# SCoulY/MuSCLe

Measured on AMD Instinct MI355X. Metric: images/sec (whole node), MCL EfficientNet-B7 448x448 bs=32/GPU, higher is better.
Workload: dtype f32; 1 GPU; train_mcl.py loop body, step-A (epoch-4 gates: focal+softmargin+pairwise+ER+IMC, one backward, one Adam step), MuSCLe(efficientnet-b7, last_pooling=False, 21 classes), random-init weights; per_gpu_batch=32, global_batch=32, image=448x448, parallelism=single, optimizer=Adam(lr=1e-4, wd=5e-5) fused, launch=eager, weight-gradient GEMMs on a second stream

## Files before the change

### include/muscle_hip.h

```cpp
#ifndef MUSCLE_HIP_H
#define MUSCLE_HIP_H

#ifdef __cplusplus
extern "C" {
#endif

int mx_version(void);
int mx_abi_hash(void);
const char* mx_last_error(void);


int mx_pw_fwd_parts(int M, int N, int K);
int mx_pw_fwd(const float* A, int a_mode, const float* a_scale, const float* a_shift, const float* a_gate,
              int rows_per_sample, const float* W, float* C, int M, int K, int N, int lda, int ldc,
              const float* bias, const float* residual, int relu, float* stats, void* stream);

int mx_set_gemm_mode(int mode);
int mx_get_gemm_mode(void);
int mx_set_wgrad_kernel(int kernel, int groups);
int mx_get_wgrad_kernel(void);
int mx_gemm_uses_split(int kind, int M, int N, int K);

long mx_pw_planes_bytes(int N, int K);
int mx_pw_planes_tiles(int N, int K);
// ... 58 lines not shown
                  const float* Wp, const float* g2, const float* b2, const float* m2, const float* v2, float eps2,
                  int Cin, int Cexp, int Cout, float* We_f, float* be, float* s1, float* t1, float* Wp_f, float* bp, void* stream);

int mx_bn_apply(const float* P, const float* scale, const float* shift, const float* row_scale, const float* residual,
                const float* gate, float* out, long rows, int C, int rows_per_sample, int act, void* stream);

int mx_bn_bwd_reduce(const float* G, const float* X, const float* row_scale, const float* gate, const float* gate_add,
                     const float* act_scale, const float* act_shift, long rows, int C, int rows_per_sample,
                     float* part, void* stream);

int mx_bn_bwd_finalize(const float* part, int P, int C, double count, const float* gamma, const float* mean, const float* rstd,
                       int training, float* dgamma, float* dbeta, float* c1, float* c2, float* c3, double* acc,
                       void* stream);

int mx_bn_bwd_apply(const float* G, const float* X, const float* row_scale, const float* gate, const float* gate_add,
                    const float* act_scale, const float* act_shift, const float* c1, const float* c2, const float* c3,
                    float* out, long rows, int C, int rows_per_sample, void* stream);

long mx_pool_ws(long rows, int C, int rows_per_sample, int planes);
int mx_pool_sum(const float* X, const float* G, const float* scale, const float* shift, int act, long rows, int C,
                int rows_per_sample, float* out, void* ws, long ws_bytes, void* stream);

int mx_se_bn1_pool(const float* dA, const float* X, const float* scale, const float* shift, long rows, int C, int rows_per_sample,
                   float* out5, void* ws, long ws_bytes, void* stream);
int mx_bn1_sums_finalize(const float* pooled5, const float* gate, const float* gh, const float* W1, float inv_hw, float* add,
                         int N, int C, int SQ, double count, const float* gamma, const float* mean, const float* rstd, int training,
                         float* dgamma, float* dbeta, float* c1, float* c2, float* c3, void* stream);


int mx_dwconv_fwd_parts(int N, int Ho, int Wo, int C, int S);
long mx_dwconv_fwd_ws(int N, int Ho, int Wo, int C, int S);
int mx_dwconv_fwd(const float* X, const float* scale, const float* shift, const float* W, float* Y, float* stats,
                  const float* pool_scale, const float* pool_shift, float* pooled, void* ws, long ws_bytes, int N,
                  int H, int Wd, int C, int K, int S, int pad_lo, int Ho, int Wo, void* stream);

int mx_dwconv_bwd_data(const float* dY, const float* W, const float* residual, float* dX, int N, int H, int Wd, int C,
                       int K, int S, int pad_lo, int Ho, int Wo, void* stream);

int mx_dwconv_bwd_weight_parts(int N, int Ho, int Wo, int C, int S);
int mx_dwconv_bwd_weight(const float* X, const float* scale, const float* shift, const float* dY, float* dW, float* dw_scratch,
                         int N, int H, int Wd, int C, int K, int S, int pad_lo, int Ho, int Wo, void* stream);

int mx_dwconv_bwd_fused_parts(int N, int H, int Wd, int C, int K);
int mx_dwconv_bwd_fused(const float* dA, const float* D, const float* gate, const float* add, const float* a1, const float* b1,
                        const float* c1, const float* c2, const float* c3, const float* X, const float* a0, const float* b0,
                        const float* W, const float* residual, float* gX, float* dW, float* dw_scratch, float* part, int N, int H,
                        int Wd, int C, int K, int pad_lo, void* stream);

int mx_dwconv_bwd_fused_bn0(const float* dA, const float* D, const float* gate, const float* add, const float* a1, const float* b1,
                            const float* c1, const float* c2, const float* c3, const float* X, const float* a0, const float* b0,
                            const float* W, float* gX, float* dW, float* dw_scratch, float* part, int N, int H, int Wd, int C, int K,
                            int pad_lo, void* ws, long ws_bytes, double count, const float* gamma, const float* mean, const float* rstd,
                            int training, float* dgamma, float* dbeta, float* o1, float* o2, float* o3, void* stream);

int mx_dw_parts_reduce(const float* part, int P, int n, float* dW, void* stream);


int mx_se_fwd(const float* pooled_sum, float inv_hw, const float* W1, const float* b1, const float* W2, const float* b2,
              float* s, float* h, float* gate, int N, int C, int SQ, void* stream);

int mx_se_bwd(const float* ggate, const float* gate, const float* s, const float* h, const float* W2,
              float* dW1, float* db1, float* dW2, float* db2, float* gh, int N, int C,
              int SQ, void* stream);

int mx_se_bwd_gh(const float* ggate, const float* gate, const float* h, const float* W2, float* gh, int N, int C, int SQ,
                 void* stream);
int mx_se_bwd_params(const float* ggate, const float* gate, const float* s, const float* h, const float* gh, float* dW1, float* db1,
                     float* dW2, float* db2, int N, int C, int SQ, void* stream);

int mx_stem_im2col(const float* img, float* out, int N, int H, int W, int Ho, int Wo, int pad_lo, void* stream);


int mx_resize_nhwc(const float* src, float* dst, int N, int Hs, int Ws, int C, int Hd, int Wd, int ldd, int coff, int relu,
                   void* stream);

int mx_upsample_to_nchw(const float* src, float* dst, int N, int Hs, int Ws, int lds, int K, int Hd, int Wd, void* stream);

int mx_infer_accum(const float* src, float* acc, int h, int w, int lds, int K, int Hs, int Ws, int H, int W, int flip, void* stream);
int mx_infer_norm(float* acc, int channels, long HW, void* stream);

int mx_cam_infer(const long* passes, int npass, int lds, int K, int H, int W, const int* keep, int nkeep, float* out_cam,
                 float* out_sgc, void* stream);

int mx_seg_infer(const long* passes, int npass, int lds, int K, int H, int W, const float* cls_scale, unsigned char* pred,
                 float* prob, void* stream);
int mx_seg_confusion(const unsigned char* pred, const unsigned char* gt, int K, int H, int W, long long* counts, void* stream);

int mx_seg_infer_batch(const long* rows, int nrow, int B, int lds, int K, int H, int W, const float* cls_scale, unsigned char* pred,
                       float* prob, const unsigned char* gt, long long* counts, void* stream);

int mx_input_stage(const unsigned char* src, const int* jobs, float* dst, int n, int Hd, int Wd, void* stream);

int mx_color_jitter(unsigned char* src, const int* jobs, unsigned long long* sums, int n, int max_pixels, void* stream);

int mx_resample(const unsigned char* src, const int* jobs, const int* tabs, unsigned char* tmp, unsigned char* dst, int n,
                int max_pixels, void* stream);

int mx_mask_stage(const void* src, const int* jobs, const int* tabs, float* dst, int n, int C, int S, int span_cap, void* stream);
int mx_seg_input_stage(const unsigned char* src, const int* jobs, float* dst, int n, int Hd, int Wd, void* stream);

int mx_irn_affinity(const float* edge, int h, int w, int radius, const int* pcoord, const int* poff, const int* plen, int nd,
                    float* dense, int ld, int n4, void* stream);
int mx_irn_transition(float* dense, int n4, int ld, float beta, float* colsum, void* stream);
int mx_irn_finish(const float* rw, int C, int h, int w, int H, int W, float bg_thres, unsigned* max_scratch, unsigned char* label,
                  void* soft_half, void* stream);
int mx_irn_walk_weights(const float* edge, int h, int w, int radius, const int* pcoord, const int* poff, const int* plen, int nd,
// ... 142 lines not shown
```

### muscle_amd/csrc/dwconv.hip

```cpp
#include "common.h"

constexpr int CB = 32;
constexpr int C4B = CB / 4;

struct DwArgs {
  const float* x;
  const float* sc;
  const float* sh;
  const float* w;
  const float* dy;
  const float* res;
  float* y;
  float* stats;
  const float* ps;
  const float* pb;
  float* pooled;
  float* poolpart;
  unsigned* counters;
  int N, H, W, Ho, Wo, C, pad;
  int tiles_x, tiles_y;
  int tiles_per_block;
  int gpp;
};

// ... 649 lines not shown
      }
      if (XAHEAD && gi + 1 < NG) {
#pragma unroll
        for (int o = 0; o < PX; ++o) xr[o] = xn[XAHEAD ? o : 0];
      }
    }
    DW_STAMP(3);
  }
  __syncthreads();
  float* slots = reinterpret_cast<float*>(td);
  const int wave = tid >> 6;
#pragma unroll
  for (int t = 0; t < K * K; ++t) {
    float2 p = part[t];
    p.x += __shfl_xor(p.x, 16, 64); p.y += __shfl_xor(p.y, 16, 64);
    p.x += __shfl_xor(p.x, 32, 64); p.y += __shfl_xor(p.y, 32, 64);
    if ((tid & 63) < C2B) *reinterpret_cast<float2*>(slots + (wave * K * K + t) * CB + 2 * c2) = p;
  }
  __syncthreads();
  for (int i = tid; i < K * K * CB; i += 256) {
    int cc = i % CB, tap = i / CB;
    if (c0 + cc < a.C)
      a.dwpart[(long)grp_id * a.C * K * K + (long)(c0 + cc) * K * K + tap] =
          ((slots[i] + slots[K * K * CB + i]) + slots[2 * K * K * CB + i]) + slots[3 * K * K * CB + i];
  }
  if (a.part) {
    __syncthreads();
#pragma unroll
    for (int o = 16; o < 64; o <<= 1) {
      s0.x += __shfl_xor(s0.x, o, 64); s0.y += __shfl_xor(s0.y, o, 64);
      s1.x += __shfl_xor(s1.x, o, 64); s1.y += __shfl_xor(s1.y, o, 64);
    }
    if ((tid & 63) < C2B) {
      *reinterpret_cast<float2*>(slots + wave * 2 * CB + 2 * c2) = s0;
      *reinterpret_cast<float2*>(slots + wave * 2 * CB + CB + 2 * c2) = s1;
    }
    __syncthreads();
    if (tid < 2 * CB) {
      const int cc = tid % CB;
      if (c0 + cc < a.C) {
        const float v = ((slots[tid] + slots[2 * CB + tid]) + slots[4 * CB + tid]) + slots[6 * CB + tid];
        float* dst = a.part + (long)grp_id * 2 * a.C + (tid / CB) * a.C + c0 + cc;
        if (a.fin_counters) mx_st_wt(dst, v); else *dst = v;
      }
    }
    if (a.fin_counters) {
      __shared__ unsigned fin_flag;
      if (mx_last_arriver(a.fin_counters + chunk_id, gridDim.x, &fin_flag))
        bn_bwd_reduce_finalize_32(a.part, (int)gridDim.x, a.C, c0, a.fin, reinterpret_cast<double*>(td));
    }
  }
}

__global__ __launch_bounds__(256) void dw_parts_reduce_kernel(const float* __restrict__ part, int P, int n, float* __restrict__ dW) {
  __shared__ float red[16][17];
  const int el = threadIdx.x & 15, gl = threadIdx.x >> 4;
  const int i = blockIdx.x * 16 + el;
  float s0 = 0.f, s1 = 0.f, s2 = 0.f, s3 = 0.f;
  if (i < n) {
    int g = gl;
    for (; g + 48 < P; g += 64) {
      s0 += part[(long)g * n + i]; s1 += part[(long)(g + 16) * n + i]; s2 += part[(long)(g + 32) * n + i]; s3 += part[(long)(g + 48) * n + i];
    }
    for (; g < P; g += 16) s0 += part[(long)g * n + i];
  }
  red[gl][el] = (s0 + s1) + (s2 + s3);
  __syncthreads();
  if (gl == 0 && i < n) {
    float t = red[0][el];
#pragma unroll
    for (int k = 1; k < 16; ++k) t += red[k][el];
    dW[i] += t;
  }
}

static void launch_dw_parts_reduce(const float* part, int P, int n, float* dW, hipStream_t st) {
  hipLaunchKernelGGL(dw_parts_reduce_kernel, dim3(cdiv(n, 16)), dim3(256), 0, st, part, P, n, dW);
}

static int dw_fused_shape(int H, int Wd, int K) {
  if (K != 5) return (Wd % 28 == 0) ? 3 : 0;
  const double small = (double)cdiv(H, 8) * cdiv(Wd, 16) * (8 + K - 1) * (16 + K - 1);
  const double large = (double)cdiv(H, 14) * cdiv(Wd, 28) * (14 + K - 1) * (28 + K - 1);
  return large < 0.9 * small ? 1 : 0;
}

static void dw_fused_geom(int N, int H, int Wd, int C, int K, int* tiles_x, int* tiles_y, int* tpb, int* groups) {
  const int shape = dw_fused_shape(H, Wd, K);
  *tiles_x = cdiv(Wd, shape ? 28 : 16); *tiles_y = cdiv(H, shape == 3 ? 8 : shape ? 14 : 8);
  const int ntile = (*tiles_x) * (*tiles_y);
  long ntiles = (long)N * ntile;
  int chunks = cdiv(C, CB);
  const long group_target = shape == 3 ? 4096 : shape ? 512 : K == 5 ? 1024 : 4096;
  long g = group_target / chunks;
  if (g < 1) g = 1;
  if (g > ntiles) g = ntiles;
  *tpb = (int)((ntiles + g - 1) / g);
  *groups = cdiv(ntiles, *tpb);
}

static int dw_check(const DwArgs& a, int K, int S, const char* who) {
  MX_CHECK_ARG(K == 3 || K == 5, "%s: kernel %d unsupported (3 or 5)", who, K);
  MX_CHECK_ARG(S == 1 || S == 2, "%s: stride %d unsupported (1 or 2)", who, S);
  MX_CHECK_ARG(a.N > 0 && a.H > 0 && a.W > 0 && a.C > 0 && a.C % 4 == 0, "%s: bad extents N=%d H=%d W=%d C=%d", who, a.N, a.H, a.W, a.C);
  MX_CHECK_ARG(a.Ho > 0 && a.Wo > 0 && (a.Ho - 1) * S + K - a.pad <= a.H + K && a.pad >= 0 && a.pad < K,
               "%s: inconsistent output size Ho=%d Wo=%d pad=%d", who, a.Ho, a.Wo, a.pad);
// ... 157 lines not shown
                           stream, nullptr, nullptr);
}

int mx_dwconv_bwd_fused_bn0(const float* dA, const float* D, const float* gate, const float* add, const float* a1, const float* b1,
                            const float* c1, const float* c2, const float* c3, const float* X, const float* a0, const float* b0,
                            const float* W, float* gX, float* dW, float* dw_scratch, float* part, int N, int H, int Wd, int C, int K,
                            int pad_lo, void* ws, long ws_bytes, double count, const float* gamma, const float* mean, const float* rstd,
                            int training, float* dgamma, float* dbeta, float* o1, float* o2, float* o3, void* stream) {
  MX_CHECK_ARG(a0 && b0 && part, "dwconv_bwd_fused_bn0: the BatchNorm-0 form only (a0, b0, part)");
  MX_CHECK_ARG(ws && ws_bytes >= MX_WS_COUNTER_BYTES && ((uintptr_t)ws & 15) == 0, "dwconv_bwd_fused_bn0: scratch with %d bytes of counters required", MX_WS_COUNTER_BYTES);
  MX_CHECK_ARG(gamma && mean && rstd && dgamma && dbeta && o1 && o2 && o3 && count > 0, "dwconv_bwd_fused_bn0: null pointer");
  MX_CHECK_ARG(cdiv(C, CB) <= MX_WS_COUNTERS, "dwconv_bwd_fused_bn0: too many channel chunks");
  BnBwdFin fin{count, gamma, mean, rstd, training, dgamma, dbeta, o1, o2, o3};
  return dw_bwd_fused_impl(dA, D, gate, add, a1, b1, c1, c2, c3, X, a0, b0, W, nullptr, gX, dW, dw_scratch, part, N, H, Wd, C, K, pad_lo,
                           stream, reinterpret_cast<unsigned*>(ws), &fin);
}

static int dw_bwd_fused_impl(const float* dA, const float* D, const float* gate, const float* add, const float* a1, const float* b1,
                            const float* c1, const float* c2, const float* c3, const float* X, const float* a0, const float* b0,
                            const float* W, const float* residual, float* gX, float* dW, float* dw_scratch, float* part, int N, int H,
                            int Wd, int C, int K, int pad_lo, void* stream, unsigned* fin_counters, const BnBwdFin* fin) {
  MX_CHECK_ARG(dA && D && gate && add && a1 && b1 && c1 && c2 && c3 && X && W && gX && dw_scratch, "dwconv_bwd_fused: null pointer");
  MX_CHECK_ARG((a0 == nullptr) == (b0 == nullptr), "dwconv_bwd_fused: a0/b0 come together");
  MX_CHECK_ARG(!a0 || part, "dwconv_bwd_fused: BN0 present -> part required");
  MX_CHECK_ARG((K == 3 || K == 5) && pad_lo == (K - 1) / 2, "dwconv_bwd_fused: stride 1 with symmetric pad only (K=%d pad=%d)", K, pad_lo);
  MX_CHECK_ARG(N > 0 && H > 0 && Wd > 0 && C > 0 && C % 4 == 0, "dwconv_bwd_fused: bad extents");
  DwFusedArgs a{};
  a.dA = dA; a.d = D; a.gate = gate; a.add = add; a.a1 = a1; a.b1 = b1; a.c1 = c1; a.c2 = c2; a.c3 = c3;
  a.x = X; a.a0 = a0; a.b0 = b0; a.w = W; a.res = residual; a.gx = gX; a.dwpart = dw_scratch; a.part = a0 ? part : nullptr;
  a.N = N; a.H = H; a.W = Wd; a.C = C; a.pad = pad_lo;
  int groups;
  dw_fused_geom(N, H, Wd, C, K, &a.tiles_x, &a.tiles_y, &a.tiles_per_block, &groups);
  dim3 grid(groups, cdiv(C, CB), 1);
  a.chunks = grid.y;
  if (fin_counters) { a.fin_counters = fin_counters; a.fin = *fin; }
  const int shape = dw_fused_shape(H, Wd, K);
  if (shape == 3) {
    hipLaunchKernelGGL((dw_bwd_fused_kernel<3, 8, 28, 7>), grid, dim3(256), 0, (hipStream_t)stream, a);
  } else if (shape) {
    if (K == 3) hipLaunchKernelGGL((dw_bwd_fused_kernel<3, 14, 28, 7>), grid, dim3(256), 0, (hipStream_t)stream, a);
    else hipLaunchKernelGGL((dw_bwd_fused_kernel<5, 14, 28, 7>), grid, dim3(256), 0, (hipStream_t)stream, a);
  } else {
    if (K == 3) hipLaunchKernelGGL((dw_bwd_fused_kernel<3, 8, 16, 8>), grid, dim3(256), 0, (hipStream_t)stream, a);
    else hipLaunchKernelGGL((dw_bwd_fused_kernel<5, 8, 16, 8>), grid, dim3(256), 0, (hipStream_t)stream, a);
  }
  MX_LAUNCH_CHECK();
  if (dW) {
    launch_dw_parts_reduce(dw_scratch, groups, C * K * K, dW, (hipStream_t)stream);
    MX_LAUNCH_CHECK();
  }
  return MX_OK;
}

int mx_dw_parts_reduce(const float* part, int P, int n, float* dW, void* stream) {
  MX_CHECK_ARG(part && dW && P > 0 && n > 0, "dw_parts_reduce: bad arguments");
  launch_dw_parts_reduce(part, P, n, dW, (hipStream_t)stream);
  MX_LAUNCH_CHECK();
  return MX_OK;
}

}
```

### muscle_amd/engine.py

```python
from __future__ import annotations

import os

from dataclasses import dataclass, field
from typing import Dict, List, Optional

import torch

from . import ops
from .arch import BlockCfg, NetCfg
from .ops import BNState


@dataclass
class BlockTape:
    cfg: BlockCfg
    H: int
    W: int
    Ho: int
    Wo: int
    x: torch.Tensor
    x_st: Optional[BNState]
    e_raw: Optional[torch.Tensor] = None
    bn0: Optional[BNState] = None
# ... 232 lines not shown
        d2 = t.d_raw.view(Mo, b.cexp)
        pooled = ops.pool_sum(d2, ho * wo, st=t.bn1, act=True)
        t.s, t.h, t.gate = ops.se_fwd(pooled, 1.0 / (ho * wo), m._se_reduce.weight.view(b.se, b.cexp), m._se_reduce.bias,
                                      m._se_expand.weight.view(b.cexp, b.se), m._se_expand.bias)
        st2 = None
        if b.cout > MATERIALISE_ABOVE:
            t.a = ops.bn_apply(d2, t.bn1, gate=t.gate, rows_per_sample=ho * wo, act=True)
            t.p_raw = ops.pw_fwd(t.a, m._project_conv.weight.view(b.cout, b.cexp), b.cout, want_stats=training,
                                 planes=tape.wp.get(id(m._project_conv.weight)))
        else:
            t.p_raw = ops.pw_fwd(d2, m._project_conv.weight.view(b.cout, b.cexp), b.cout, a_mode=ops.BNACT,
                                 a_scale=t.bn1.scale, a_shift=t.bn1.shift, a_gate=t.gate, rows_per_sample=ho * wo,
                                 want_stats=training, planes=tape.wp.get(id(m._project_conv.weight)))
        if training:
            t.p_raw, st2 = t.p_raw
        t.bn2 = ops.bn_finalize(st2, Mo, m._bn2, training)
        if b.skip and training and b.drop_rate:
            if drop_u is not None:
                keep = 1.0 - b.drop_rate
                t.row_scale = torch.floor(keep + drop_u[b.index].to(dev, torch.float32)) / keep
            else:
                t.row_scale = drop_scales[b.index]
        res = None
        if b.skip:
            assert x_st is None
            res = x.view(M, b.cin)
        t.out = ops.bn_apply(t.p_raw, t.bn2, row_scale=t.row_scale, residual=res, rows_per_sample=ho * wo).view(N, ho, wo, b.cout)
        tape.blocks.append(t)
        x, x_st, h, w = t.out, None, ho, wo
        if not save:
            t.x = t.e_raw = t.d_raw = t.p_raw = t.a = None
            if b.index == 0:
                tape.cols = tape.stem_raw = None
            if len(tape.blocks) >= 2 and tape.blocks[-2].cfg.index not in cfg.taps:
                tape.blocks[-2].out = None
    ops.flush_batch_counters()
    return tape


class GradSink:

    def __init__(self):
        self.bufs: Dict[int, torch.Tensor] = {}

    def of(self, p: torch.nn.Parameter) -> torch.Tensor:
        g = self.bufs.get(id(p))
        if g is None:
            g = torch.zeros_like(p, memory_format=torch.contiguous_format)
            self.bufs[id(p)] = g
        return g


FOLD_BN0_EARLY = os.environ.get("MUSCLE_FOLD_BN0_EARLY", "1") == "1"
WGRAD_SIDE_STREAM = os.environ.get("MUSCLE_WGRAD_STREAM", "1") == "1"
_side_streams: Dict[int, "torch.cuda.Stream"] = {}


class _WgradLane:
    def __init__(self, device):
        self.s = None
        self.pending = []
        self.keep = []
        if WGRAD_SIDE_STREAM:
            key = device.index if device.index is not None else torch.cuda.current_device()
            if key not in _side_streams:
                _side_streams[key] = torch.cuda.Stream(device=device)
            self.s = _side_streams[key]

    def _queue(self, launch, *reads):
        if self.s is None:
            return launch()
        self.pending.append((launch, reads))

    def wgrad(self, G, X, dW, **kw):
        return self._queue(lambda: ops.pw_wgrad(G, X, dW, **kw), G, X)

    def wgrad_bnbwd(self, G, G2, coef, X, dW):
        return self._queue(lambda: ops.pw_wgrad_bnbwd(G, G2, coef, X, dW), G, X, G2, coef)

    def dw_reduce(self, scratch, dW):
        return self._queue(lambda: ops.dw_parts_reduce(scratch, dW), scratch)

    def flush(self):
        if self.s is None or not self.pending:
            return
        self.s.wait_stream(torch.cuda.current_stream())
        with torch.cuda.stream(self.s):
            for launch, _ in self.pending:
                launch()
        self.keep.extend(reads for _, reads in self.pending)
        self.pending = []

    def progress(self, done, module):
        if self.s is None:
            return done(module)
        self.flush()
        self.s.wait_stream(torch.cuda.current_stream())
        with torch.cuda.stream(self.s):
            done(module)

    def join(self):
        self.flush()
        if self.s is not None:
            torch.cuda.current_stream().wait_stream(self.s)
        self.keep = []


def _dw_input(t: BlockTape):
    return (t.e_raw, t.bn0) if t.cfg.expand else (t.x, t.x_st)


def _project_backward(lane, tape: Tape, t: BlockTape, m, g_out, sink: GradSink):
    b, hw = t.cfg, t.Ho * t.Wo
    Mo = tape.N * hw
    dp = ops.bn_backward(g_out.reshape(Mo, b.cout), t.p_raw, m._bn2, t.bn2, sink.of(m._bn2.weight), sink.of(m._bn2.bias), tape.training,
                         row_scale=t.row_scale, rows_per_sample=hw)
    if t.a is not None:
        lane.wgrad(dp, t.a, sink.of(m._project_conv.weight).view(b.cout, b.cexp))
        t.a = None
    else:
        lane.wgrad(dp, t.d_raw.view(Mo, b.cexp), sink.of(m._project_conv.weight).view(b.cout, b.cexp), x_mode=ops.BNACT,
                   x_scale=t.bn1.scale, x_shift=t.bn1.shift, x_gate=t.gate, rows_per_sample=hw)
    ga = ops.pw_dgrad(dp, m._project_conv.weight.view(b.cout, b.cexp), b.cexp, wt=tape.wt.get(id(m._project_conv.weight)),
                      planes=tape.wtp.get(id(m._project_conv.weight)))
    lane.flush()
    return ga


def _se_bn1_coeffs(tape: Tape, t: BlockTape, m, ga, sink: GradSink):
    b, hw = t.cfg, t.Ho * t.Wo
    Mo = tape.N * hw
    pooled5 = ops.se_bn1_pool(ga, t.d_raw.view(Mo, b.cexp), t.bn1, hw)
    gh = ops.se_bwd(pooled5[0], t.gate, t.s, t.h, m._se_expand.weight.view(b.cexp, b.se),
                    sink.of(m._se_reduce.weight).view(b.se, b.cexp), sink.of(m._se_reduce.bias),
                    sink.of(m._se_expand.weight).view(b.cexp, b.se), sink.of(m._se_expand.bias))
    return ops.bn1_coeffs(pooled5, t.gate, gh, m._se_reduce.weight.view(b.se, b.cexp), 1.0 / hw, Mo, m._bn1, t.bn1,
                          sink.of(m._bn1.weight), sink.of(m._bn1.bias), tape.training)


def _depthwise_backward(lane, tape: Tape, t: BlockTape, m, ga, c1, add, skip_res, sink: GradSink):
    b, N = t.cfg, tape.N
    dw_in, dw_st = _dw_input(t)
    res = None if dw_st is not None else skip_res
    if b.stride == 1 and b.pad_lo == (b.kernel - 1) // 2:
        return ops.dwconv_bwd_fused(ga.view(N, t.Ho, t.Wo, b.cexp), t.d_raw, t.gate, add, t.bn1, c1, dw_in, dw_st,
                                    m._depthwise_conv.weight, sink.of(m._depthwise_conv.weight), b.kernel, b.pad_lo,
                                    residual=res, defer=lane.dw_reduce)
    dd = ops.bn_backward_from_coeffs(ga, t.d_raw.view(N * t.Ho * t.Wo, b.cexp), t.bn1, c1, gate=t.gate, gate_add=add,
                                     rows_per_sample=t.Ho * t.Wo, out=ga).view(N, t.Ho, t.Wo, b.cexp)
    ops.dwconv_bwd_weight(dw_in, dd, sink.of(m._depthwise_conv.weight), b.kernel, b.stride, b.pad_lo, st=dw_st)
    return ops.dwconv_bwd_data(dd, m._depthwise_conv.weight, b.kernel, b.stride, b.pad_lo, t.H, t.W, residual=res), None


def _bn0_expand_backward(lane, backbone, cfg: NetCfg, tape: Tape, t: BlockTape, m, gx, part0, skip_res, sink: GradSink):
    b, N, training = t.cfg, tape.N, tape.training
    dw_in, dw_st = _dw_input(t)
    bn_mod = m._bn0 if b.expand else backbone._bn0
    M = N * t.H * t.W
    raw2, gx2 = dw_in.view(M, dw_in.shape[3]), gx.view(M, dw_in.shape[3])
    res = skip_res.reshape(M, b.cin) if skip_res is not None else None
    if part0 is not None:
        c0 = ops.bn_bwd_coeffs(part0, M, bn_mod, dw_st, sink.of(bn_mod.weight), sink.of(bn_mod.bias), training)
        wtp = tape.wtp.get(id(m._expand_conv.weight)) if b.expand else None
        if FOLD_BN0_EARLY and wtp is not None and ops.bnbwd_fold_takes(M, b.cexp, b.cin) == "small":
            lane.wgrad_bnbwd(gx2, raw2, c0, t.x.view(M, b.cin), sink.of(m._expand_conv.weight).view(b.cexp, b.cin))
            g_in = ops.pw_dgrad_bnbwd_planes(gx2, raw2, c0, wtp, b.cin, residual=res)
            lane.flush()
            return g_in.view(N, t.H, t.W, b.cin)
        dz = ops.bn_bwd_apply_plain(gx2, raw2, c0, gx2)
    else:
        dz = ops.bn_backward(gx2, raw2, bn_mod, dw_st, sink.of(bn_mod.weight), sink.of(bn_mod.bias), training, act=dw_st, out=gx2)
    if not b.expand:
        dw28 = torch.zeros(cfg.stem_out, 28, dtype=torch.float32, device=dz.device)
        ops.pw_wgrad(dz, tape.cols, dw28)
        sink.of(backbone._conv_stem.weight).view(cfg.stem_out, 27).add_(dw28[:, :27])
        return None
    lane.wgrad(dz, t.x.view(M, b.cin), sink.of(m._expand_conv.weight).view(b.cexp, b.cin))
    g_in = ops.pw_dgrad(dz, m._expand_conv.weight.view(b.cexp, b.cin), b.cin, wt=tape.wt.get(id(m._expand_conv.weight)),
                        planes=tape.wtp.get(id(m._expand_conv.weight)), residual=res)
    lane.flush()
    return g_in.view(N, t.H, t.W, b.cin)


def backbone_backward(backbone, cfg: NetCfg, tape: Tape, tap_grads: Dict[int, torch.Tensor], sink: GradSink):
    g_out: Optional[torch.Tensor] = None
    lane = _WgradLane(tape.blocks[0].out.device)
    if tape.wt_event is not None:
        torch.cuda.current_stream().wait_event(tape.wt_event)
    done = getattr(sink, "block_done", None) if getattr(sink, "on_ready", None) is not None else None
    for t in reversed(tape.blocks):
        m = _blk(backbone, t.cfg.index)
        tg = tap_grads.get(t.cfg.index)
        if tg is not None:
            g_out = tg if g_out is None else g_out + tg
        if g_out is None:
            continue
        ga = _project_backward(lane, tape, t, m, g_out, sink)
        c1, add = _se_bn1_coeffs(tape, t, m, ga, sink)
        skip_res = g_out if t.cfg.skip else None
        gx, part0 = _depthwise_backward(lane, tape, t, m, ga, c1, add, skip_res, sink)
        del ga
        if _dw_input(t)[1] is not None:
            g_out = _bn0_expand_backward(lane, backbone, cfg, tape, t, m, gx, part0, skip_res, sink)
        else:
            g_out = gx
        if done is not None:
            lane.progress(done, m)
    lane.join()
```

### muscle_amd/ops.py

```python
from __future__ import annotations

import os
from typing import NamedTuple, Optional

import torch

from ._lib import call, lib, ptr, stream

PLAIN, BNACT, AFFINE = 0, 1, 2


class BNState(NamedTuple):
    scale: torch.Tensor
    shift: torch.Tensor
    mean: torch.Tensor
    rstd: torch.Tensor


def _f32(*shape, device):
    return torch.empty(shape, dtype=torch.float32, device=device)


_scratch_bufs: dict = {}
_wgrad_ws: dict = {}
# ... 376 lines not shown
    return out


def bn_bwd_coeffs(part, rows, bn, st: BNState, dgamma, dbeta, training: bool):
    P, _, C = part.shape
    c = _f32(3, C, device=part.device)
    base = c.data_ptr()
    call("mx_bn_bwd_finalize", ptr(part), P, C, float(rows), ptr(bn.weight), ptr(st.mean), ptr(st.rstd), int(training),
         ptr(dgamma), ptr(dbeta), base, base + 4 * C, base + 8 * C, _acc_scratch(part.device, 128 * C), stream())
    return c


def bn_bwd_apply_plain(G2d, X2d, c, out):
    rows, C = X2d.shape
    cb, cs = c.data_ptr(), 4 * c.shape[1]
    call("mx_bn_bwd_apply", ptr(G2d), ptr(X2d), None, None, None, None, None, cb, cb + cs, cb + 2 * cs, ptr(out),
         rows, C, 1, stream())
    return out


def dw_parts_reduce(scratch, dW):
    P, n = scratch.shape
    call("mx_dw_parts_reduce", ptr(scratch), P, n, ptr(dW), stream())


def dwconv_bwd_fused(dA, D, gate, add, st1: BNState, c1, X, st0: Optional[BNState], W, dW, K, pad_lo, *, residual=None, defer=None,
                     bn0=None):
    N, H, Wd, C = X.shape
    gX = _f32(N, H, Wd, C, device=X.device)
    P = lib().mx_dwconv_bwd_fused_parts(N, H, Wd, C, K)
    part = _f32(P, 2, C, device=X.device) if st0 is not None else None
    scratch = _f32(P, C * K * K, device=X.device)
    cb, cs = c1.data_ptr(), 4 * c1.shape[1]
    if bn0 is not None and st0 is not None and residual is None:
        bn, dgamma, dbeta, training = bn0
        co = _f32(3, C, device=X.device)
        ob = co.data_ptr()
        ws, wsn = _scratch(X.device, 65536)
        _call_ws("mx_dwconv_bwd_fused_bn0", ptr(dA), ptr(D), ptr(gate), ptr(add), ptr(st1.scale), ptr(st1.shift), cb, cb + cs, cb + 2 * cs,
                 ptr(X), ptr(st0.scale), ptr(st0.shift), ptr(W), ptr(gX), None if defer is not None else ptr(dW), ptr(scratch), ptr(part),
                 N, H, Wd, C, K, pad_lo, ws, wsn, float(N * H * Wd), ptr(bn.weight), ptr(st0.mean), ptr(st0.rstd), int(training),
                 ptr(dgamma), ptr(dbeta), ob, ob + 4 * C, ob + 8 * C, stream())
        if defer is not None:
            defer(scratch, dW)
        return gX, part, co
    call("mx_dwconv_bwd_fused", ptr(dA), ptr(D), ptr(gate), ptr(add), ptr(st1.scale), ptr(st1.shift), cb, cb + cs,
         cb + 2 * cs, ptr(X), ptr(st0.scale) if st0 else None, ptr(st0.shift) if st0 else None, ptr(W), ptr(residual), ptr(gX),
         None if defer is not None else ptr(dW), ptr(scratch), ptr(part), N, H, Wd, C, K, pad_lo, stream())
    if defer is not None:
        defer(scratch, dW)
    return (gX, part, None) if bn0 is not None else (gX, part)


def se_bn1_pool(dA2d, X2d, st: BNState, rows_per_sample):
    rows, C = X2d.shape
    N = rows // rows_per_sample
    out = _f32(5, N, C, device=X2d.device)
    ws, wsn = _scratch(X2d.device, lib().mx_pool_ws(rows, C, rows_per_sample, 5))
    _call_ws("mx_se_bn1_pool", ptr(dA2d), ptr(X2d), ptr(st.scale), ptr(st.shift), rows, C, rows_per_sample, ptr(out), ws, wsn, stream())
    return out


def bn1_coeffs(pooled5, gate, gh, W1, inv_hw, rows, bn, st: BNState, dgamma, dbeta, training: bool):
    _, N, C = pooled5.shape
    SQ = W1.shape[0]
    c = _f32(3, C, device=gate.device)
    add = torch.empty_like(gate)
    base = c.data_ptr()
    call("mx_bn1_sums_finalize", ptr(pooled5), ptr(gate), ptr(gh), ptr(W1), float(inv_hw), ptr(add), N, C, SQ, float(rows),
         ptr(bn.weight), ptr(st.mean), ptr(st.rstd), int(training), ptr(dgamma), ptr(dbeta), base, base + 4 * C, base + 8 * C, stream())
    return c, add


def pool_sum(X2d, rows_per_sample, *, G=None, st: Optional[BNState] = None, act=False):
    rows, C = X2d.shape
    out = _f32(rows // rows_per_sample, C, device=X2d.device)
    ws, wsn = _scratch(X2d.device, lib().mx_pool_ws(rows, C, rows_per_sample, 1))
    _call_ws("mx_pool_sum", ptr(X2d), ptr(G), ptr(st.scale) if st else None, ptr(st.shift) if st else None, int(act), rows, C,
             rows_per_sample, ptr(out), ws, wsn, stream())
    return out


def dwconv_fwd(X, W, K, S, pad_lo, Ho, Wo, *, st: Optional[BNState] = None, want_stats=False, pool=None):
    N, H, Wd, C = X.shape
    Y = _f32(N, Ho, Wo, C, device=X.device)
    stats = _f32(lib().mx_dwconv_fwd_parts(N, Ho, Wo, C, S), 2, C, device=X.device) if want_stats else None
    pooled = _f32(N, C, device=X.device) if pool is not None else None
    ws, wsn = _scratch(X.device, lib().mx_dwconv_fwd_ws(N, Ho, Wo, C, S)) if pool is not None else (None, 0)
    _call_ws("mx_dwconv_fwd", ptr(X), ptr(st.scale) if st else None, ptr(st.shift) if st else None, ptr(W), ptr(Y), ptr(stats),
             ptr(pool[0]) if pool is not None else None, ptr(pool[1]) if pool is not None else None, ptr(pooled), ws, wsn,
             N, H, Wd, C, K, S, pad_lo, Ho, Wo, stream())
    if pool is not None:
        return Y, pooled
    return (Y, stats) if want_stats else Y


def dwconv_bwd_data(dY, W, K, S, pad_lo, H, Wd, *, residual=None):
    N, Ho, Wo, C = dY.shape
    dX = _f32(N, H, Wd, C, device=dY.device)
    call("mx_dwconv_bwd_data", ptr(dY), ptr(W), ptr(residual), ptr(dX), N, H, Wd, C, K, S, pad_lo, Ho, Wo, stream())
    return dX


def dwconv_bwd_weight(X, dY, dW, K, S, pad_lo, *, st: Optional[BNState] = None):
    N, H, Wd, C = X.shape
    _, Ho, Wo, _ = dY.shape
# ... 234 lines not shown
```

Measured before the change: 340.8 images/sec.

## Add fused depthwise-conv backward kernel for stride-2 blocks

Adds a stride-2 variant of the fused depthwise backward kernel. It folds the BN1/swish/SE-gate backward, the input-gradient convolution, the BN0 swish recomputation, the weight-gradient partials and the BN0 reduction partials into one tiled pass. Before this, stride-2 blocks ran a separate BN backward, dwconv weight-grad and data-grad kernels. The aim is fewer full-tensor round trips through memory for the downsampling blocks. The early BN0 fold path is also restricted to stride-1 so that stride-2 blocks use the new partials, and the new kernel adds register and LDS pressure.

```diff
diff --git a/include/muscle_hip.h b/include/muscle_hip.h
--- a/include/muscle_hip.h
+++ b/include/muscle_hip.h
@@ -134,6 +134,12 @@
                             const float* W, float* gX, float* dW, float* dw_scratch, float* part, int N, int H, int Wd, int C, int K,
                             int pad_lo, void* ws, long ws_bytes, double count, const float* gamma, const float* mean, const float* rstd,
                             int training, float* dgamma, float* dbeta, float* o1, float* o2, float* o3, void* stream);
+
+int mx_dwconv_bwd_fused_s2_parts(int N, int H, int Wd, int C, int K);
+int mx_dwconv_bwd_fused_s2(const float* dA, const float* D, const float* gate, const float* add, const float* a1, const float* b1,
+                           const float* c1, const float* c2, const float* c3, const float* X, const float* a0, const float* b0,
+                           const float* W, float* gX, float* dW, float* dw_scratch, float* part, int N, int H, int Wd, int C, int K,
+                           int pad_lo, int Ho, int Wo, void* stream);
 
 int mx_dw_parts_reduce(const float* part, int P, int n, float* dW, void* stream);
 
diff --git a/muscle_amd/csrc/dwconv.hip b/muscle_amd/csrc/dwconv.hip
--- a/muscle_amd/csrc/dwconv.hip
+++ b/muscle_amd/csrc/dwconv.hip
@@ -725,6 +725,196 @@
   }
 }
 
+struct DwFusedS2Args {
+  const float* dA; const float* d;
+  const float* gate; const float* add;
+  const float* a1; const float* b1;
+  const float* c1; const float* c2; const float* c3;
+  const float* x; const float* a0; const float* b0;
+  const float* w;
+  float* gx; float* dwpart; float* part;
+  int N, H, W, Ho, Wo, C, pad, tiles_x, tiles_y, tiles_per_block;
+};
+
+template <int K>
+__global__ __launch_bounds__(256, K == 3 ? 3 : 2) void dw_bwd_fused_s2_kernel(DwFusedS2Args a) {
+  constexpr int TH = 8, TW = 32, HK = (K - 1) / 2;
+  constexpr int OH = TH / 2 + HK, OW = TW / 2 + HK, OWP = OW | 1;
+  constexpr int TOT = OH * OW * C4B, PER = (TOT + 255) / 256;
+  constexpr int C2B = CB / 2, PX = 8, QB = PX / 2;
+  static_assert((TH / 2) * (TW / PX) * C2B == 256, "thread mapping");
+  __shared__ float4 td[OH * OWP * C4B];
+  static_assert(OH * OWP * C4B * 4 >= 4 * K * K * CB, "the per-wave partial rows reuse the staged tile");
+  __shared__ __attribute__((aligned(16))) float wl[K * K * CB];
+  __shared__ __attribute__((aligned(16))) float cst[9 * CB];
+  const int tid = threadIdx.x, c0 = blockIdx.y * CB;
+  const int c4 = tid % C4B;
+  const int c = c0 + 4 * c4;
+  const bool cok = c < a.C;
+  const int c2 = tid % C2B, pq = tid / C2B;
+  const int rp = pq % (TH / 2), seg = pq / (TH / 2);
+  const int cc2 = c0 + 2 * c2;
+  const bool cok2 = cc2 < a.C;
+  const int ntile = a.tiles_x * a.tiles_y;
+  const long t_beg = (long)blockIdx.x * a.tiles_per_block;
+  const long t_end = min((long)a.N * ntile, t_beg + a.tiles_per_block);
+  for (int i = tid; i < K * K * CB; i += 256) {
+    int cc = i % CB, tap = i / CB;
+    wl[i] = (c0 + cc < a.C) ? a.w[(long)(c0 + cc) * K * K + tap] : 0.f;
+  }
+  for (int i = tid; i < 7 * CB; i += 256) {
+    int cc = i % CB, j = i / CB;
+    const float* src = j == 0 ? a.a1 : j == 1 ? a.b1 : j == 2 ? a.c1 : j == 3 ? a.c2 : j == 4 ? a.c3 : j == 5 ? a.a0 : a.b0;
+    cst[i] = (c0 + cc < a.C) ? src[c0 + cc] : 0.f;
+  }
+  float2 part[K * K];
+#pragma unroll
+  for (int t = 0; t < K * K; ++t) part[t] = make_float2(0, 0);
+  float2 s0 = make_float2(0, 0), s1 = s0;
+  const int par = a.pad & 1;
+  for (long t = t_beg; t < t_end; ++t) {
+    const int n = (int)(t / ntile), rem = (int)(t % ntile);
+    const int iy0 = (rem / a.tiles_x) * TH - par, ix0 = (rem % a.tiles_x) * TW - par;
+    const int oy_lo = (iy0 + a.pad) / 2 - HK, ox_lo = (ix0 + a.pad) / 2 - HK;
+    __syncthreads();
+    if (tid < 2 * CB) {
+      int cc = tid % CB;
+      cst[7 * CB + tid] = (c0 + cc < a.C) ? (tid < CB ? a.gate : a.add)[(long)n * a.C + c0 + cc] : 0.f;
+    }
+    float2 xr[2][PX];
+    const int iyb = iy0 + 2 * rp, ixb = ix0 + PX * seg;
+#pragma unroll
+    for (int pu = 0; pu < 2; ++pu) {
+      const float* row = a.x + (((long)n * a.H + min(max(iyb + pu, 0), a.H - 1)) * a.W) * a.C + (cok2 ? cc2 : 0);
+#pragma unroll
+      for (int j = 0; j < PX; ++j) xr[pu][j] = *reinterpret_cast<const float2*>(row + min(max(ixb + j, 0), a.W - 1) * a.C);
+    }
+    __syncthreads();
+    {
+      float4 vg[PER], vd[PER];
+      unsigned okm = 0;
+#pragma unroll
+      for (int k = 0; k < PER; ++k) {
+        const int i = min(tid + 256 * k, TOT - 1), pix = i / C4B;
+        int oy = oy_lo + pix / OW, ox = ox_lo + pix % OW;
+        okm |= (oy >= 0 && oy < a.Ho && ox >= 0 && ox < a.Wo && cok) ? (1u << k) : 0u;
+        oy = min(max(oy, 0), a.Ho - 1); ox = min(max(ox, 0), a.Wo - 1);
+        const long off = (((long)n * a.Ho + oy) * a.Wo + ox) * a.C + (cok ? c : 0);
+        vg[k] = ld4(a.dA + off); vd[k] = ld4(a.d + off);
+      }
+      const float4 A1 = ld4(cst + 4 * c4), B1 = ld4(cst + CB + 4 * c4), C1 = ld4(cst + 2 * CB + 4 * c4),
+                   C2 = ld4(cst + 3 * CB + 4 * c4), C3 = ld4(cst + 4 * CB + 4 * c4),
+                   G = ld4(cst + 7 * CB + 4 * c4), AD = ld4(cst + 8 * CB + 4 * c4);
+#define DD1(f) dd.f = okf * (C1.f * ((vg[k].f * G.f + AD.f) * swish_gradf_(A1.f * vd[k].f + B1.f)) + C2.f * vd[k].f + C3.f);
+#pragma unroll
+      for (int k = 0; k < PER; ++k) {
+        const int i = min(tid + 256 * k, TOT - 1), pix = i / C4B;
+        const float okf = ((okm >> k) & 1u) ? 1.f : 0.f;
+        float4 dd;
+        DD1(x) DD1(y) DD1(z) DD1(w)
+        td[((pix / OW) * OWP + pix % OW) * C4B + c4] = dd;
+      }
+#undef DD1
+    }
+    __syncthreads();
+    const float2 A0 = *reinterpret_cast<const float2*>(cst + 5 * CB + 2 * c2), B0 = *reinterpret_cast<const float2*>(cst + 6 * CB + 2 * c2);
+    const float2* tdg = reinterpret_cast<const float2*>(td) + (rp * OWP + seg * QB) * C2B + c2;
+    const float2* wl2 = reinterpret_cast<const float2*>(wl) + c2;
+#pragma unroll
+    for (int pu = 0; pu < 2; ++pu) {
+      const int iy = iyb + pu;
+      const bool rok = cok2 && iy >= 0 && iy < a.H;
+      float2 xa[PX], df[PX], ah[PX];
+      bool img[PX];
+#pragma unroll
+      for (int j = 0; j < PX; ++j) {
+        const float2 r = xr[pu][j];
+        img[j] = rok && ixb + j >= 0 && ixb + j < a.W;
+        const float zx = A0.x * r.x + B0.x, zy = A0.y * r.y + B0.y;
+        const float sx = sigmoidf_(zx), sy = sigmoidf_(zy);
+        xa[j] = img[j] ? make_float2(zx * sx, zy * sy) : make_float2(0.f, 0.f);
+        df[j] = make_float2(sx * (1.0f + zx * (1.0f - sx)), sy * (1.0f + zy * (1.0f - sy)));
+        ah[j] = make_float2(0.f, 0.f);
+      }
+#pragma unroll
+      for (int m = 0; pu + 2 * m < K; ++m) {
+        const int ky = pu + 2 * m;
+        float2 in[QB + HK];
+#pragma unroll
+        for (int q = 0; q < QB + HK; ++q) in[q] = tdg[((HK - m) * OWP + q) * C2B];
+#pragma unroll
+        for (int kx = 0; kx < K; ++kx) {
+          const int pv = kx & 1, mx = kx >> 1;
+          const float2 w = wl2[(ky * K + kx) * C2B];
+          float2& p = part[ky * K + kx];
+#pragma unroll
+          for (int jb = 0; jb < QB; ++jb) {
+            const float2 v = in[jb + HK - mx];
+            const int j = 2 * jb + pv;
+            ah[j].x += w.x * v.x; ah[j].y += w.y * v.y;
+            p.x += xa[j].x * v.x; p.y += xa[j].y * v.y;
+          }
+        }
+      }
+      const long rowoff = (((long)n * a.H + min(max(iy, 0), a.H - 1)) * a.W) * a.C + cc2;
+#pragma unroll
+      for (int j = 0; j < PX; ++j) {
+        if (img[j]) {
+          const float2 r = xr[pu][j];
+          float2 v = ah[j];
+          v.x *= df[j].x; v.y *= df[j].y;
+          s0.x += v.x; s0.y += v.y;
+          s1.x += v.x * r.x; s1.y += v.y * r.y;
+          *reinterpret_cast<float2*>(a.gx + rowoff + (long)(ixb + j) * a.C) = v;
+        }
+      }
+    }
+  }
+  __syncthreads();
+  float* slots = reinterpret_cast<float*>(td);
+  const int wave = tid >> 6;
+#pragma unroll
+  for (int t = 0; t < K * K; ++t) {
+    float2 p = part[t];
+    p.x += __shfl_xor(p.x, 16, 64); p.y += __shfl_xor(p.y, 16, 64);
+    p.x += __shfl_xor(p.x, 32, 64); p.y += __shfl_xor(p.y, 32, 64);
+    if ((tid & 63) < C2B) *reinterpret_cast<float2*>(slots + (wave * K * K + t) * CB + 2 * c2) = p;
+  }
+  __syncthreads();
+  for (int i = tid; i < K * K * CB; i += 256) {
+    int cc = i % CB, tap = i / CB;
+    if (c0 + cc < a.C)
+      a.dwpart[(long)blockIdx.x * a.C * K * K + (long)(c0 + cc) * K * K + tap] =
+          ((slots[i] + slots[K * K * CB + i]) + slots[2 * K * K * CB + i]) + slots[3 * K * K * CB + i];
+  }
+  __syncthreads();
+#pragma unroll
+  for (int o = 16; o < 64; o <<= 1) {
+    s0.x += __shfl_xor(s0.x, o, 64); s0.y += __shfl_xor(s0.y, o, 64);
+    s1.x += __shfl_xor(s1.x, o, 64); s1.y += __shfl_xor(s1.y, o, 64);
+  }
+  if ((tid & 63) < C2B) {
+    *reinterpret_cast<float2*>(slots + wave * 2 * CB + 2 * c2) = s0;
+    *reinterpret_cast<float2*>(slots + wave * 2 * CB + CB + 2 * c2) = s1;
+  }
+  __syncthreads();
+  if (tid < 2 * CB) {
+    const int cc = tid % CB;
+    if (c0 + cc < a.C)
+      a.part[(long)blockIdx.x * 2 * a.C + (tid / CB) * a.C + c0 + cc] =
+          ((slots[tid] + slots[2 * CB + tid]) + slots[4 * CB + tid]) + slots[6 * CB + tid];
+  }
+}
+
+static int dw_fused_s2_groups(int N, int H, int Wd, int C, int K) {
+  const long ntiles = (long)N * cdiv(Wd, 32) * cdiv(H, 8);
+  long g = (K == 5 ? 2048 : 4096) / cdiv(C, CB);
+  if (g > 1024) g = 1024;
+  if (g < 1) g = 1;
+  if (g > ntiles) g = ntiles;
+  return cdiv(ntiles, cdiv(ntiles, g));
+}
+
 __global__ __launch_bounds__(256) void dw_parts_reduce_kernel(const float* __restrict__ part, int P, int n, float* __restrict__ dW) {
   __shared__ float red[16][17];
   const int el = threadIdx.x & 15, gl = threadIdx.x >> 4;
@@ -988,6 +1178,40 @@
   return MX_OK;
 }
 
+int mx_dwconv_bwd_fused_s2_parts(int N, int H, int Wd, int C, int K) {
+  if (N <= 0 || H <= 0 || Wd <= 0 || C <= 0 || (K != 3 && K != 5)) return MX_EARG;
+  return dw_fused_s2_groups(N, H, Wd, C, K);
+}
+
+int mx_dwconv_bwd_fused_s2(const float* dA, const float* D, const float* gate, const float* add, const float* a1, const float* b1,
+                           const float* c1, const float* c2, const float* c3, const float* X, const float* a0, const float* b0,
+                           const float* W, float* gX, float* dW, float* dw_scratch, float* part, int N, int H, int Wd, int C, int K,
+                           int pad_lo, int Ho, int Wo, void* stream) {
+  MX_CHECK_ARG(a0 && b0, "dwconv_bwd_fused_s2: the BatchNorm-0 form only (a0, b0 required)");
+  MX_CHECK_ARG(dA && D && gate && add && a1 && b1 && c1 && c2 && c3 && X && W && gX && dw_scratch && part, "dwconv_bwd_fused_s2: null pointer");
+  MX_CHECK_ARG(K == 3 || K == 5, "dwconv_bwd_fused_s2: kernel %d unsupported (3 or 5)", K);
+  MX_CHECK_ARG(N > 0 && H > 0 && Wd > 0 && C > 0 && C % 4 == 0, "dwconv_bwd_fused_s2: bad extents N=%d H=%d W=%d C=%d", N, H, Wd, C);
+  MX_CHECK_ARG((pad_lo == (K - 1) / 2 || pad_lo == (K - 1) / 2 - 1) && Ho > 0 && Wo > 0 && (Ho - 1) * 2 + K - pad_lo <= H + K &&
+               (Wo - 1) * 2 + K - pad_lo <= Wd + K,
+               "dwconv_bwd_fused_s2: inconsistent static same padding / output size (K=%d pad=%d H=%d W=%d Ho=%d Wo=%d)", K, pad_lo, H, Wd, Ho, Wo);
+  DwFusedS2Args a{};
+  a.dA = dA; a.d = D; a.gate = gate; a.add = add; a.a1 = a1; a.b1 = b1; a.c1 = c1; a.c2 = c2; a.c3 = c3;
+  a.x = X; a.a0 = a0; a.b0 = b0; a.w = W; a.gx = gX; a.dwpart = dw_scratch; a.part = part;
+  a.N = N; a.H = H; a.W = Wd; a.Ho = Ho; a.Wo = Wo; a.C = C; a.pad = pad_lo;
+  a.tiles_x = cdiv(Wd + (pad_lo & 1), 32); a.tiles_y = cdiv(H + (pad_lo & 1), 8);
+  const int groups = dw_fused_s2_groups(N, H, Wd, C, K);
+  a.tiles_per_block = cdiv((long)N * a.tiles_x * a.tiles_y, groups);
+  dim3 grid(groups, cdiv(C, CB), 1);
+  if (K == 3) hipLaunchKernelGGL((dw_bwd_fused_s2_kernel<3>), grid, dim3(256), 0, (hipStream_t)stream, a);
+  else hipLaunchKernelGGL((dw_bwd_fused_s2_kernel<5>), grid, dim3(256), 0, (hipStream_t)stream, a);
+  MX_LAUNCH_CHECK();
+  if (dW) {
+    launch_dw_parts_reduce(dw_scratch, groups, C * K * K, dW, (hipStream_t)stream);
+    MX_LAUNCH_CHECK();
+  }
+  return MX_OK;
+}
+
 int mx_dw_parts_reduce(const float* part, int P, int n, float* dW, void* stream) {
   MX_CHECK_ARG(part && dW && P > 0 && n > 0, "dw_parts_reduce: bad arguments");
   launch_dw_parts_reduce(part, P, n, dW, (hipStream_t)stream);
diff --git a/muscle_amd/engine.py b/muscle_amd/engine.py
--- a/muscle_amd/engine.py
+++ b/muscle_amd/engine.py
@@ -308,6 +308,7 @@
 
 
 FOLD_BN0_EARLY = os.environ.get("MUSCLE_FOLD_BN0_EARLY", "1") == "1"
+DW_S2_FUSED = os.environ.get("MUSCLE_DW_S2_FUSED", "1") == "1"
 WGRAD_SIDE_STREAM = os.environ.get("MUSCLE_WGRAD_STREAM", "1") == "1"
 _side_streams: Dict[int, "torch.cuda.Stream"] = {}
 
@@ -402,6 +403,10 @@
         return ops.dwconv_bwd_fused(ga.view(N, t.Ho, t.Wo, b.cexp), t.d_raw, t.gate, add, t.bn1, c1, dw_in, dw_st,
                                     m._depthwise_conv.weight, sink.of(m._depthwise_conv.weight), b.kernel, b.pad_lo,
                                     residual=res, defer=lane.dw_reduce)
+    if DW_S2_FUSED and b.stride == 2 and dw_st is not None:
+        return ops.dwconv_bwd_fused_s2(ga.view(N, t.Ho, t.Wo, b.cexp), t.d_raw, t.gate, add, t.bn1, c1, dw_in, dw_st,
+                                       m._depthwise_conv.weight, sink.of(m._depthwise_conv.weight), b.kernel, b.pad_lo,
+                                       defer=lane.dw_reduce)
     dd = ops.bn_backward_from_coeffs(ga, t.d_raw.view(N * t.Ho * t.Wo, b.cexp), t.bn1, c1, gate=t.gate, gate_add=add,
                                      rows_per_sample=t.Ho * t.Wo, out=ga).view(N, t.Ho, t.Wo, b.cexp)
     ops.dwconv_bwd_weight(dw_in, dd, sink.of(m._depthwise_conv.weight), b.kernel, b.stride, b.pad_lo, st=dw_st)
@@ -418,7 +423,7 @@
     if part0 is not None:
         c0 = ops.bn_bwd_coeffs(part0, M, bn_mod, dw_st, sink.of(bn_mod.weight), sink.of(bn_mod.bias), training)
         wtp = tape.wtp.get(id(m._expand_conv.weight)) if b.expand else None
-        if FOLD_BN0_EARLY and wtp is not None and ops.bnbwd_fold_takes(M, b.cexp, b.cin) == "small":
+        if FOLD_BN0_EARLY and b.stride == 1 and wtp is not None and ops.bnbwd_fold_takes(M, b.cexp, b.cin) == "small":
             lane.wgrad_bnbwd(gx2, raw2, c0, t.x.view(M, b.cin), sink.of(m._expand_conv.weight).view(b.cexp, b.cin))
             g_in = ops.pw_dgrad_bnbwd_planes(gx2, raw2, c0, wtp, b.cin, residual=res)
             lane.flush()
diff --git a/muscle_amd/ops.py b/muscle_amd/ops.py
--- a/muscle_amd/ops.py
+++ b/muscle_amd/ops.py
@@ -452,6 +452,22 @@
     return (gX, part, None) if bn0 is not None else (gX, part)
 
 
+def dwconv_bwd_fused_s2(dA, D, gate, add, st1: BNState, c1, X, st0: BNState, W, dW, K, pad_lo, *, defer=None):
+    N, H, Wd, C = X.shape
+    _, Ho, Wo, _ = D.shape
+    gX = _f32(N, H, Wd, C, device=X.device)
+    P = lib().mx_dwconv_bwd_fused_s2_parts(N, H, Wd, C, K)
+    part = _f32(P, 2, C, device=X.device)
+    scratch = _f32(P, C * K * K, device=X.device)
+    cb, cs = c1.data_ptr(), 4 * c1.shape[1]
+    call("mx_dwconv_bwd_fused_s2", ptr(dA), ptr(D), ptr(gate), ptr(add), ptr(st1.scale), ptr(st1.shift), cb, cb + cs, cb + 2 * cs,
+         ptr(X), ptr(st0.scale), ptr(st0.shift), ptr(W), ptr(gX), None if defer is not None else ptr(dW), ptr(scratch), ptr(part),
+         N, H, Wd, C, K, pad_lo, Ho, Wo, stream())
+    if defer is not None:
+        defer(scratch, dW)
+    return gX, part
+
+
 def se_bn1_pool(dA2d, X2d, st: BNState, rows_per_sample):
     rows, C = X2d.shape
     N = rows // rows_per_sample
```

New measurement: 344.6 images/sec (median of 6 runs). 1.1% higher.
